# colmap/glomap

Measured on NVIDIA B200. Metric: observations/sec per BA LM-iteration, higher is better.
Workload: dtype f64

## Files before the change

### glomap_b200/csrc/ba_kernels.cuh

```cuda
#pragma once
#include "common.cuh"
#include "pcg.cuh"

namespace b200 {

constexpr int kCamRec = 8;
constexpr int kIntrRec = 8;
constexpr double kZEps = 1e-12;
constexpr int kSeg = 256;
constexpr int kIntrSmem = 16;
constexpr int kJpDoubles = 6;
constexpr int kJcDoubles = 9;
constexpr int kSensorRec = 16;

struct BAView {
  int C, P, K;
  long long N;
  int n_tiles;
  int n_segs;
  int min_views;
  const int* obs_cam;
  const int* obs_pt;
  const double2* obs_xy;
  const unsigned* pt_begin;
// ... 489 lines not shown
  }
  const double d = U[(size_t)c * 21 + sym_idx(6, k, k)];
  const double js2 = js * js;
  Dc[i] = fmin(fmax(d * js2, 1e-6), 1e32) / (radius * js2);
}

__device__ __forceinline__ void point_damping(const double* V6, const double* js, double radius, double Dp[3]) {
  const double d[3] = {V6[0], V6[3], V6[5]};
#pragma unroll
  for (int k = 0; k < 3; ++k) {
    const double js2 = js[k] * js[k];
    Dp[k] = fmin(fmax(d[k] * js2, 1e-6), 1e32) / (radius * js2);
  }
}
__global__ void ba_damp_points(int P, const double* __restrict__ V, double* __restrict__ jscale_p, int set_jscale,
                               double radius, double* __restrict__ Vinv) {
  const int p = blockIdx.x * blockDim.x + threadIdx.x;
  if (p >= P) return;
  double v6[6];
#pragma unroll
  for (int k = 0; k < 6; ++k) v6[k] = V[6 * (size_t)p + k];
  double js[3];
  if (set_jscale) {
    js[0] = 1.0 / (1.0 + sqrt(v6[0]));
    js[1] = 1.0 / (1.0 + sqrt(v6[3]));
    js[2] = 1.0 / (1.0 + sqrt(v6[5]));
#pragma unroll
    for (int k = 0; k < 3; ++k) jscale_p[3 * (size_t)p + k] = js[k];
  } else {
#pragma unroll
    for (int k = 0; k < 3; ++k) js[k] = jscale_p[3 * (size_t)p + k];
  }
  double Dp[3];
  point_damping(v6, js, radius, Dp);
  v6[0] += Dp[0];
  v6[3] += Dp[1];
  v6[5] += Dp[2];
  double inv[6];
  sym3_inverse(v6, inv);
#pragma unroll
  for (int k = 0; k < 6; ++k) Vinv[6 * (size_t)p + k] = inv[k];
}

__global__ void __launch_bounds__(128) ba_schur_diag(BAView v) {
  const int warp = (blockIdx.x * blockDim.x + threadIdx.x) >> 5;
  const int lane = threadIdx.x & 31;
  if (warp >= v.n_segs) return;
  const int cam = v.seg_cam[warp];
  const int b = v.seg_begin[warp], e = v.seg_end[warp];
  double S[21];
#pragma unroll
  for (int k = 0; k < 21; ++k) S[k] = 0.0;
  for (int i = b + lane; i < e; i += 32) {
    const int o = v.camord_obs[i];
    const int pt = v.pt_c[i];
    double w[18], vi[6];
// ... 392 lines not shown
```

### glomap_b200/csrc/ba_kernels_v2.cuh

```cuda
#pragma once
#include "ba_kernels.cuh"
#include "pcg.cuh"

namespace b200 {

struct BAViewV2 {
  const double* Ap;
  double* Ac;
  double* z4;
  double* Bc = nullptr;
  double* Ufk = nullptr;
  const IntrVarRec* ivar = nullptr;
  int C = 0;
};

template <int NK>
__device__ __forceinline__ void obs_intr_rows(const ObsCore& o, const double* __restrict__ ir, const IntrVarRec& iv,
                                              const double Jp[6], double Jk[2][NK > 0 ? NK : 1],
                                              double B[NK > 0 ? 3 * NK : 1]) {
#pragma unroll
  for (int j = 0; j < NK; ++j) {
    double jx = 0.0, jy = 0.0;
    if (j < iv.mb) intr_param_jac(ir, iv.pidx[j], o.uv[0], o.uv[1], 1.0, jx, jy);
    if (!o.valid) jx = jy = 0.0;
// ... 187 lines not shown
      }
    }
  }
#pragma unroll
  for (int k = 0; k < 21; ++k) {
    const double s = warp_sum(U[k]);
    if (lane == k && s != 0.0) atomicAdd(&v.U[(size_t)cam * 21 + k], s);
  }
#pragma unroll
  for (int k = 0; k < 6; ++k) {
    const double s = warp_sum(g[k]);
    if (lane == 21 + k && s != 0.0) atomicAdd(&v.gc[(size_t)cam * 6 + k], s);
  }
}

__global__ void __launch_bounds__(128) ba2_schur_diag(BAView v, BAViewV2 v2, const double* __restrict__ cam_rec) {
  const int warp = (blockIdx.x * blockDim.x + threadIdx.x) >> 5;
  const int lane = threadIdx.x & 31;
  if (warp >= v.n_segs) return;
  const int cam = v.seg_cam[warp];
  const int b = v.seg_begin[warp], e = v.seg_end[warp];
  double RR[6] = {0, 0, 0, 0, 0, 0}, RT[9] = {0, 0, 0, 0, 0, 0, 0, 0, 0}, TT[6] = {0, 0, 0, 0, 0, 0};
  const double* row = v2.Ac + (size_t)(v.seg_row0[warp] >> 5) * (kJcDoubles * 32) + lane;
  for (int i = b + lane; i < e; i += 32, row += kJcDoubles * 32) {
    const double A[6] = {ld_stream(row), ld_stream(row + 32), ld_stream(row + 64), ld_stream(row + 96), ld_stream(row + 128),
                         ld_stream(row + 160)};
    const double X[3] = {ld_stream(row + 192), ld_stream(row + 224), ld_stream(row + 256)};
    const int pt = ld_stream(v.pt_c + i);
    const double2* vp = reinterpret_cast<const double2*>(v.Vinv + (size_t)pt * 6);
    const double2 v0 = vp[0], v1 = vp[1], v2_ = vp[2];
    const double vi[6] = {v0.x, v0.y, v1.x, v1.y, v2_.x, v2_.y};
    const double Ac0[3] = {A[0], A[1], A[2]}, Ac1[3] = {A[1], A[3], A[4]}, Ac2[3] = {A[2], A[4], A[5]};
    double T0[3], T1[3], T2[3];
    sym3_mul(vi, Ac0, T0);
    sym3_mul(vi, Ac1, T1);
    sym3_mul(vi, Ac2, T2);
    double N[3][3];
    {
      double c0[3], c1[3], c2[3];
      sym3_mul(A, T0, c0);
      sym3_mul(A, T1, c1);
      sym3_mul(A, T2, c2);
#pragma unroll
      for (int r = 0; r < 3; ++r) { N[r][0] = c0[r]; N[r][1] = c1[r]; N[r][2] = c2[r]; }
    }
// ... 14 lines not shown
    }
    RR[0] += -2.0 * PK[0][0]; RR[1] += -2.0 * PK[0][1]; RR[2] += -2.0 * PK[0][2];
    RR[3] += -2.0 * PK[1][1]; RR[4] += -2.0 * PK[1][2]; RR[5] += -2.0 * PK[2][2];
#pragma unroll
    for (int r = 0; r < 3; ++r)
#pragma unroll
      for (int c = 0; c < 3; ++c) RT[3 * r + c] += P[r][c];
    TT[0] += N[0][0]; TT[1] += N[0][1]; TT[2] += N[0][2]; TT[3] += N[1][1]; TT[4] += N[1][2]; TT[5] += N[2][2];
  }
#pragma unroll
  for (int k = 0; k < 6; ++k) RR[k] = warp_sum(RR[k]);
#pragma unroll
  for (int k = 0; k < 9; ++k) RT[k] = warp_sum(RT[k]);
#pragma unroll
  for (int k = 0; k < 6; ++k) TT[k] = warp_sum(TT[k]);
  if (lane == 0) {
    const double4 q4c = ld_rec32(cam_rec + (size_t)cam * kCamRec);
    const double4 t4c = ld_rec32(cam_rec + (size_t)cam * kCamRec + 4);
    const int mask = (int)(__double_as_longlong(t4c.w) & 0xff);
    const double q[4] = {q4c.x, q4c.y, q4c.z, q4c.w};
    double R[9];
    quat_to_R(q, R);
    double M[6][6];
    const double rr[3][3] = {{RR[0], RR[1], RR[2]}, {RR[1], RR[3], RR[4]}, {RR[2], RR[4], RR[5]}};
    const double tt[3][3] = {{TT[0], TT[1], TT[2]}, {TT[1], TT[3], TT[4]}, {TT[2], TT[4], TT[5]}};
    for (int r = 0; r < 3; ++r)
      for (int c = 0; c < 3; ++c) {
        M[r][c] = rr[r][c];
        M[3 + r][3 + c] = tt[r][c];
        M[r][3 + c] = RT[3 * r + c];
        M[3 + c][r] = RT[3 * r + c];
      }
    double T[6][6];
    for (int blk = 0; blk < 2; ++blk)
      for (int r = 0; r < 3; ++r)
        for (int c = 0; c < 6; ++c)
          T[3 * blk + r][c] = R[3 * r] * M[3 * blk][c] + R[3 * r + 1] * M[3 * blk + 1][c] + R[3 * r + 2] * M[3 * blk + 2][c];
// ... 170 lines not shown
  for (long long r = (long long)blockIdx.x * blockDim.x + threadIdx.x; r < rows; r += (long long)gridDim.x * blockDim.x) {
    const double2* row = reinterpret_cast<const double2*>(part + 4 * r);
    const double2 u = row[0], w = row[1];
    a0 += u.x; a1 += u.y; a2 += w.x; a3 += w.y;
  }
  a0 = block_sum(a0, scratch);
  a1 = block_sum(a1, scratch);
  a2 = block_sum(a2, scratch);
  a3 = block_sum(a3, scratch);
  if (threadIdx.x == 0) {
    double* o = out + 4 * (size_t)blockIdx.x;
    o[0] = a0; o[1] = a1; o[2] = a2; o[3] = a3;
  }
}

__global__ void ba2_point_rhs_z(BAView v, BAViewV2 v2) {
  const int p = blockIdx.x * blockDim.x + threadIdx.x;
  if (p >= v.P) return;
  double vi[6], g[3], z[3];
#pragma unroll
  for (int k = 0; k < 6; ++k) vi[k] = v.Vinv[6 * (size_t)p + k];
#pragma unroll
  for (int k = 0; k < 3; ++k) g[k] = v.gp[3 * (size_t)p + k];
  sym3_mul(vi, g, z);
  const bool pvalid = (int)(v.pt_begin[p + 1] - v.pt_begin[p]) >= v.min_views;
  *reinterpret_cast<double4*>(v2.z4 + 4 * (size_t)p) = pvalid ? make_double4(z[0], z[1], z[2], 0.0) : make_double4(0, 0, 0, 0);
}

template <int NK>
__global__ void __launch_bounds__(128, B200_PB_MIN_CTAS) ba2_pass_b(BAView v, BAViewV2 v2, const double* __restrict__ cam_rec,
                                                 double* __restrict__ y, const PcgCtl* __restrict__ ctl, int seg_lo,
                                                 int seg_hi) {
  if (ctl && ctl->done) return;
  const int warp = seg_lo + ((blockIdx.x * blockDim.x + threadIdx.x) >> 5);
  const int lane = threadIdx.x & 31;
  if (warp >= seg_hi) return;
  const int cam = v.seg_cam[warp];
  const int b = v.seg_begin[warp], e = v.seg_end[warp];
  double acc[6] = {0, 0, 0, 0, 0, 0};
  constexpr int NKK = NK > 0 ? NK : 1;
  double accK[NKK];
#pragma unroll
  for (int k = 0; k < NKK; ++k) accK[k] = 0.0;
// ... 157 lines not shown
```

### glomap_b200/csrc/ba_kernels_v3.cuh

```cuda
#pragma once
#include "ba_kernels_v2.cuh"

namespace b200 {

constexpr int kEllWindow = 1024;
constexpr int kEllThreads = 128;

struct EllView {
  int n_groups;
  const int* row0;
  const int* pt;
  const int* len;
  const int* cam;
  const double2* xy;
  const unsigned short* sensor;
  double* A;
  double* B = nullptr;
};

template <class Sort>
__global__ void __launch_bounds__(kEllWindow) ell_sort_window(int P, int min_views, const unsigned* __restrict__ pt_begin,
                                                              int* __restrict__ ell_pt, int* __restrict__ ell_len,
                                                              int* __restrict__ ell_slot, int* __restrict__ group_rows) {
  __shared__ typename Sort::TempStorage tmp;
// ... 181 lines not shown
#pragma unroll
      for (int k = 0; k < 3; ++k) {
        v.gp[3 * (size_t)pt + k] = gp[k];
        gmax = fmax(gmax, fabs(gp[k]));
      }
    }
  }
  cost = warp_sum(cost);
  gmax = warp_max(gmax);
  if (lane == 0) {
    part_cost[slot >> 5] = cost;
    part_gmax[slot >> 5] = gmax;
  }
}

__global__ void __launch_bounds__(kEllThreads) ba3_cost(BAView v, EllView ell, const double* __restrict__ cam_rec,
                                                         const double* __restrict__ intr_rec,
                                                         const double* __restrict__ points, double huber_a,
                                                         double* __restrict__ part_cost) {
  __shared__ double scratch[32];
  const int slot = blockIdx.x * kEllThreads + threadIdx.x;
  const int lane = threadIdx.x & 31;
  const int g = slot >> 5;
  double cost = 0.0;
  if (g < ell.n_groups) {
    const int pt = ell.pt[slot];
    const int mylen = ell.len[slot];
    const int r0 = ell.row0[g], nrow = ell.row0[g + 1] - r0;
    double X0 = 0, X1 = 0, X2 = 0;
    if (pt >= 0) {
      X0 = points[3 * (size_t)pt]; X1 = points[3 * (size_t)pt + 1]; X2 = points[3 * (size_t)pt + 2];
    }
#pragma unroll 2
    for (int j = 0; j < nrow; ++j) {
      if (j >= mylen) continue;
      const size_t idx = ((size_t)r0 + j) * 32 + lane;
      const int cam = ld_stream(ell.cam + idx);
      const double2 xy = ld_stream(ell.xy + idx);
      const double4 q4 = ld_rec32(cam_rec + (size_t)cam * kCamRec);
      const double4 t4 = ld_rec32(cam_rec + (size_t)cam * kCamRec + 4);
      const double* sr = ell.sensor ? v.sensor_rec + (size_t)ell.sensor[idx] * kSensorRec : nullptr;
      const double* ir = intr_rec + (size_t)obs_intr_idx(t4, sr) * kIntrRec;
      const double q[4] = {q4.x, q4.y, q4.z, q4.w};
      double R[9];
      quat_to_R(q, R);
      double xc = R[0] * X0 + R[1] * X1 + R[2] * X2 + t4.x;
      double yc = R[3] * X0 + R[4] * X1 + R[5] * X2 + t4.y;
      double zc = R[6] * X0 + R[7] * X1 + R[8] * X2 + t4.z;
      if (sr) sensor_apply(sr, xc, yc, zc);
      if (zc > kZEps) {
        double px, py;
        project_only(ir, xc, yc, zc, px, py);
        const double e0 = px - xy.x, e1 = py - xy.y;
        double rho0, rho1;
        huber(e0 * e0 + e1 * e1, huber_a, rho0, rho1);
        cost += 0.5 * rho0;
      }
    }
  }
  cost = block_sum(cost, scratch);
  if (threadIdx.x == 0) part_cost[blockIdx.x] = cost;
}

__global__ void __launch_bounds__(1024) ba3_reduce_partials(int n, const double* __restrict__ part_a,
                                                           const double* __restrict__ part_b, double* __restrict__ out_sum,
                                                           double* __restrict__ out_max) {
  __shared__ double scratch[32];
  double s = 0.0, m = 0.0;
  for (int i = threadIdx.x; i < n; i += blockDim.x) {
    s += part_a[i];
    if (part_b) m = fmax(m, part_b[i]);
  }
  s = block_sum(s, scratch);
  if (threadIdx.x == 0) *out_sum = s;
  if (part_b) {
    m = block_max(m, scratch);
    if (threadIdx.x == 0) *out_max = m;
  }
}

template <int MODE, int NK>
__global__ void __launch_bounds__(kEllThreads, MODE == 0 ? B200_EA_MIN_CTAS : B200_EA2_MIN_CTAS) ba3_pass_a(
    BAView v, EllView ell, BAViewV2 v2, const double* __restrict__ xp, const double* __restrict__ points,
    double* __restrict__ points_new, double radius, double* __restrict__ bscal, const PcgCtl* __restrict__ ctl) {
  __shared__ double scratch[32];
  if (ctl && ctl->done) return;
  const int slot = blockIdx.x * kEllThreads + threadIdx.x;
  const int lane = threadIdx.x & 31;
  const int g = slot >> 5;
  double b0 = 0, b1 = 0, b2 = 0, b3 = 0;
  if (g < ell.n_groups) {
    const int pt = ell.pt[slot];
// ... 93 lines not shown
```

### glomap_b200/csrc/ba_solver.cuh

```cuda
#pragma once
#include <cub/cub.cuh>

#include <algorithm>
#include <cmath>
#include <cstdlib>
#include <vector>

#include "ba_kernels.cuh"
#include "ba_kernels_v2.cuh"
#include "ba_kernels_v3.cuh"
#include "ba_kernels_ext.cuh"
#include "filter_kernels.cuh"
#include "processor_kernels.cuh"
#include "context.cuh"
#include "pcg.cuh"

namespace b200 {

__global__ void k_expand_obs_pt(int P, const unsigned* __restrict__ pt_begin, int* __restrict__ obs_pt) {
  const int p = blockIdx.x * blockDim.x + threadIdx.x;
  if (p >= P) return;
  for (unsigned o = pt_begin[p]; o < pt_begin[p + 1]; ++o) obs_pt[o] = p;
}
__global__ void k_cam_keys(long long N, int VC, int smul, int min_views, const int* __restrict__ obs_cam,
// ... 107 lines not shown
  std::vector<unsigned char> h_sensor_var;
  DevBuf<unsigned char> sensor_var;
  DevBuf<double> sens_q[2], sens_t[2], sens_q_saved, sens_t_saved;
  b200::ExtView ext_view() {
    b200::ExtView e;
    e.C = C; e.K = K; e.S = S; e.ivar = ivar.p; e.sensor_var = (ext_s && S > 0) ? sensor_var.p : nullptr;
    return e;
  }
  bool use_v2 = false;
  bool use_ell = false;
  int ell_groups = 0, ell_ctas = 0, ell_bpart_rows = 0;
  long long ell_rows = 0;
  DevBuf<int> ell_row0, ell_pt, ell_len, ell_slot, ell_cam;
  DevBuf<double2> ell_xy;
  DevBuf<unsigned short> ell_sensor;
  DevBuf<double> ell_A, ell_part;
  b200::EllView ell_view() {
    b200::EllView e;
    e.n_groups = ell_groups; e.row0 = ell_row0.p; e.pt = ell_pt.p; e.len = ell_len.p; e.cam = ell_cam.p; e.xy = ell_xy.p;
    e.sensor = S > 0 ? ell_sensor.p : nullptr; e.A = ell_A.p; e.B = kfast ? ell_B.p : nullptr;
    return e;
  }
  DevBuf<double> Jc, z4, xq, bpart, bpart2;
  size_t smem_k3v2 = 0;
  bool kfast = false;
  int nk = 0;
  DevBuf<double> ell_B, Bc, Ufk;
  b200::BAViewV2 view2() {
    b200::BAViewV2 w;
    w.Ap = W.p; w.Ac = Jc.p; w.z4 = z4.p;
    w.Bc = kfast ? Bc.p : nullptr; w.Ufk = kfast ? Ufk.p : nullptr; w.ivar = ivar.p; w.C = C;
// ... 193 lines not shown
      size_t need = 0;
      cub::DeviceScan::ExclusiveSum(nullptr, need, grows.p, ell_row0.p, ell_groups + 1, s);
      DevBuf<unsigned char> tmp3;
      tmp3.alloc(need + 16);
      size_t tb3 = tmp3.bytes();
      cub::DeviceScan::ExclusiveSum(tmp3.p, tb3, grows.p, ell_row0.p, ell_groups + 1, s);
      ctx->launches += 1;
      int h_rows = 0;
      B200_CUDA_OK(cudaMemcpyAsync(&h_rows, ell_row0.p + ell_groups, sizeof(int), cudaMemcpyDeviceToHost, s));
      B200_CUDA_OK(cudaStreamSynchronize(s));
      ell_rows = h_rows;
      const size_t cells = (size_t)std::max<long long>(ell_rows, 1) * 32;
      ell_cam.alloc(cells); ell_xy.alloc(cells); ell_A.alloc(cells * 6);
      if (S > 0) ell_sensor.alloc(cells);
      ell_part.alloc((size_t)ell_ctas * (kEllThreads / 32) * 2 + 8);
      ell_bpart_rows = ell_ctas;
      B200_LAUNCH(ctx, ell_scatter_obs, cdiv(N, 256), 256, 0, N, min_views, obs_pt.p, pt_begin.p, obs_cam.p, obs_xy.p,
                  S > 0 ? obs_sensor.p : nullptr, ell_slot.p, ell_row0.p, ell_cam.p, ell_xy.p, S > 0 ? ell_sensor.p : nullptr);
      B200_CUDA_OK(cudaStreamSynchronize(s));
    }
    for (int i = 0; i < 2; ++i) {
      quat[i].alloc((size_t)C * 4); trans[i].alloc((size_t)C * 3); points[i].alloc((size_t)P * 3);
    }
    intr.alloc((size_t)K * B200SFM_INTR_STRIDE);
    intr_cand.alloc((size_t)K * B200SFM_INTR_STRIDE);
    cam_rec.alloc((size_t)C * kCamRec); intr_rec.alloc((size_t)K * kIntrRec);
    W.alloc((size_t)N * kWDoubles); V.alloc((size_t)P * 6); Vinv.alloc((size_t)P * 6); gp.alloc((size_t)P * 3);
    lin.alloc((size_t)CB * 27 + 1 + (size_t)ctx->world);
    Sd.alloc((size_t)CB * 27);
    Minv.alloc((size_t)CB * 21);
// ... 83 lines not shown
    if (S > 0)
      B200_LAUNCH(ctx, bax_build_sensor_rec, cdiv(S, 256), 256, 0, S, sens_q[which].p, sens_t[which].p,
                  sensor_intr.p, sensor_rec.p);
  }
  void set_sensor_variable(const uint8_t* h_var) {
    h_sensor_var.assign(h_var, h_var + S);
    sensor_var.upload(h_sensor_var.data(), S, ctx->stream);
    B200_CUDA_OK(cudaStreamSynchronize(ctx->stream));
  }
  void get_sensor_poses(double* h_q, double* h_t) {
    if (h_q) sens_q[cur].download(h_q, (size_t)S * 4, ctx->stream);
    if (h_t) sens_t[cur].download(h_t, (size_t)S * 3, ctx->stream);
    B200_CUDA_OK(cudaStreamSynchronize(ctx->stream));
  }

  void launch_cost(int which, double huber_a) {
    using namespace b200;
    if (use_ell) {
      B200_LAUNCH(ctx, ba3_cost, ell_ctas, kEllThreads, 0, view(), ell_view(), cam_rec.p, intr_rec.p, points[which].p, huber_a, ell_part.p);
      B200_LAUNCH(ctx, ba3_reduce_partials, 1, 256, 0, ell_ctas, ell_part.p, nullptr, scal.p + 6, nullptr);
    } else {
      const int grid = std::min(cdiv(N, 256), 148 * 8);
      B200_LAUNCH(ctx, ba_cost, grid, 256, 0, view(), cam_rec.p, intr_rec.p, points[which].p, huber_a, scal.p + 6);
    }
  }

  double eval_cost(int which, double huber_a) {
    using namespace b200;
    build_records(which);
    B200_CUDA_OK(cudaMemsetAsync(scal.p + 6, 0, sizeof(double), ctx->stream));
    launch_cost(which, huber_a);
    ctx->allreduce_sum(scal.p + 6, 1);
    B200_CUDA_OK(cudaMemcpyAsync(ctx->h_scal, scal.p + 6, sizeof(double), cudaMemcpyDeviceToHost, ctx->stream));
    B200_CUDA_OK(cudaStreamSynchronize(ctx->stream));
    return ctx->h_scal[0];
// ... 9 lines not shown
    cudaEvent_t e0 = nullptr, e1 = nullptr;
    if (profile) {
      e0 = timer_lin.next();
      e1 = timer_lin.next();
      B200_CUDA_OK(cudaEventRecord(e0, s));
    }
    if (use_ell) {
      const int nwp = ell_ctas * (kEllThreads / 32);
#define B200_LIN_P(NKV)                                                                                                   \
  B200_LAUNCH(ctx, ba3_linearize_points<NKV>, ell_ctas, kEllThreads, 0, v, ell_view(), cam_rec.p, intr_rec.p, points[cur].p, \
              huber_a, points_var ? 1 : 0, ell_part.p, ell_part.p + nwp, ivar.p)
      if (kfast && nk == 2) B200_LIN_P(2);
      else if (kfast && nk == 1) B200_LIN_P(1);
      else B200_LIN_P(0);
#undef B200_LIN_P
      B200_LAUNCH(ctx, ba3_reduce_partials, 1, 1024, 0, nwp, ell_part.p, ell_part.p + nwp, scal.p, scal.p + 1);
    } else if (use_v2)
      B200_LAUNCH(ctx, ba_linearize_points<true>, n_tiles, kTile, smem_k1, v, cam_rec.p, intr_rec.p, points[cur].p, huber_a,
                  points_var ? 1 : 0, scal.p);
    else
      B200_LAUNCH(ctx, ba_linearize_points<false>, n_tiles, kTile, smem_k1, v, cam_rec.p, intr_rec.p, points[cur].p, huber_a,
                  points_var ? 1 : 0, scal.p);
    if (profile) B200_CUDA_OK(cudaEventRecord(e1, s));
    if (n_segs > 0) {
      const int sgrid = cdiv((long long)n_segs * 32, 128);
      if (kfast) {
        Ufk.zero(s);
        B200_LAUNCH(ctx, ba2_pad_points, cdiv(P, 256), 256, 0, P, points[cur].p, z4.p);
        if (nk == 2) B200_LAUNCH(ctx, ba2_linearize_cams<2>, sgrid, 128, 0, v, view2(), cam_rec.p, intr_rec.p, points[cur].p, huber_a);
        else B200_LAUNCH(ctx, ba2_linearize_cams<1>, sgrid, 128, 0, v, view2(), cam_rec.p, intr_rec.p, points[cur].p, huber_a);
      } else if (ext) {
// ... 157 lines not shown
      else if (ext_s) B200_EXT_B(false, true);
      else B200_EXT_B(false, false);
#undef B200_EXT_B
    }
  }

  void launch_pass_b(const b200::BAView& v, double* y, const b200::PcgCtl* ctl, int seg_lo = 0, int seg_hi = -1) {
    using namespace b200;
    if (seg_hi < 0) seg_hi = n_segs;
    if (seg_hi <= seg_lo) return;
    const int grid = cdiv((long long)(seg_hi - seg_lo) * 32, 128);
    if (kfast && nk == 2) B200_LAUNCH(ctx, ba2_pass_b<2>, grid, 128, 0, v, view2(), cam_rec.p, y, ctl, seg_lo, seg_hi);
    else if (kfast) B200_LAUNCH(ctx, ba2_pass_b<1>, grid, 128, 0, v, view2(), cam_rec.p, y, ctl, seg_lo, seg_hi);
    else B200_LAUNCH(ctx, ba2_pass_b<0>, grid, 128, 0, v, view2(), cam_rec.p, y, ctl, seg_lo, seg_hi);
  }
  void launch_pass_a0(const b200::BAView& v, double radius, const b200::PcgCtl* ctl) {
    using namespace b200;
    if (kfast && nk == 2)
      B200_LAUNCH(ctx, (ba3_pass_a<0, 2>), ell_ctas, kEllThreads, 0, v, ell_view(), view2(), xq.p, points[cur].p, nullptr, radius, nullptr, ctl);
    else if (kfast)
      B200_LAUNCH(ctx, (ba3_pass_a<0, 1>), ell_ctas, kEllThreads, 0, v, ell_view(), view2(), xq.p, points[cur].p, nullptr, radius, nullptr, ctl);
    else
      B200_LAUNCH(ctx, (ba3_pass_a<0, 0>), ell_ctas, kEllThreads, 0, v, ell_view(), view2(), xq.p, points[cur].p, nullptr, radius, nullptr, ctl);
  }
  void launch_cross(const double* x, double* y, const b200::PcgCtl* ctl) {
    using namespace b200;
    if (nk == 2) B200_LAUNCH(ctx, ba2k_cross<2>, cdiv(C, 256), 256, 0, C, K, cam_rec.p, Ufk.p, x, y, ctl);
    else B200_LAUNCH(ctx, ba2k_cross<1>, cdiv(C, 256), 256, 0, C, K, cam_rec.p, Ufk.p, x, y, ctl);
  }

  StepResult compute_step(const b200sfm_ba_opts& o, double radius, bool points_var, bool set_jscale_p, bool profile) {
    using namespace b200;
    cudaStream_t s = ctx->stream;
    BAView v = view();
    const int nB6 = nbk * 6;
    if (points_var) B200_LAUNCH(ctx, ba_damp_points, cdiv(P, 256), 256, 0, P, V.p, jscale_p.p, set_jscale_p ? 1 : 0, radius, Vinv.p);
    B200_LAUNCH(ctx, ba_damp_cams, cdiv(nB6, 256), 256, 0, nbk, U(), jscale_c.p, radius, Dc.p);
    const bool recomp = ext && !kfast;
    const bool schur_jacobi = points_var && o.preconditioner == 1 && !recomp;
    double* yrhs = Sd.p + (size_t)CB * 21;
    Sd.zero(s);
    if (schur_jacobi && n_segs > 0) {
      if (use_v2) B200_LAUNCH(ctx, ba2_schur_diag, cdiv((long long)n_segs * 32, 128), 128, 0, v, view2(), cam_rec.p);
      else B200_LAUNCH(ctx, ba_schur_diag, cdiv((long long)n_segs * 32, 128), 128, 0, v);
    }
    if (points_var) {
      if (use_v2) {
        B200_LAUNCH(ctx, ba2_point_rhs_z, cdiv(P, 256), 256, 0, v, view2());
        if (recomp) ext_matvec(nullptr, yrhs, o.thres_loss_function, radius, true, nullptr);
        else if (n_segs > 0) launch_pass_b(v, yrhs, nullptr);
      } else {
        B200_LAUNCH(ctx, ba_schur_pass<1>, n_tiles, kTile, smem_k3, v, nullptr, yrhs, nullptr, nullptr, radius, nullptr);
      }
    } else if (recomp) {
      z4.zero(s);
    }
    if (schur_jacobi || points_var) ctx->allreduce_sum(Sd.p, (size_t)CB * 27);
    B200_LAUNCH(ctx, ba_build_precond, cdiv(nbk, 128), 128, 0, nbk, U(), Dc.p, schur_jacobi ? Sd.p : nullptr, Minv.p);
    B200_LAUNCH(ctx, k_rhs, cdiv(nB6, 256), 256, 0, nB6, gc(), points_var ? yrhs : nullptr, bvec.p);
    const int max_it = std::max(1, o.pcg_max_iterations);
    const int nblk = cdiv(nbk, kPcgThreads);
    ctx->pcgh.ensure(max_it, (size_t)nblk * 3, ctx->world);
    double* part_pq = ctx->pcgh.d_part;
    double* part_rz = ctx->pcgh.d_part + nblk;
// ... 272 lines not shown
```

### glomap_b200/csrc/common.cuh

```cuda
#pragma once
#include <cuda_runtime.h>
#include <stdint.h>
#include <stdio.h>

#include <string>

namespace b200 {

#ifndef B200_TILE
#define B200_TILE 128
#endif
#ifndef B200_K1_MIN_CTAS
#define B200_K1_MIN_CTAS 5
#endif
#ifndef B200_K3_MIN_CTAS
#define B200_K3_MIN_CTAS 8
#endif
#ifndef B200_PA_MIN_CTAS
#define B200_PA_MIN_CTAS 12
#endif
#ifndef B200_LC_MIN_CTAS
#define B200_LC_MIN_CTAS 3
#endif
#ifndef B200_PB_PREFETCH
#define B200_PB_PREFETCH 1
#endif
#ifndef B200_PB_MIN_CTAS
#define B200_PB_MIN_CTAS 7
#endif
#ifndef B200_E1_MIN_CTAS
#define B200_E1_MIN_CTAS 4
#endif
#ifndef B200_E1_PIPE
#define B200_E1_PIPE 1
#endif
#ifndef B200_EA_MIN_CTAS
#define B200_EA_MIN_CTAS 8
#endif
#ifndef B200_EA2_MIN_CTAS
#define B200_EA2_MIN_CTAS 6
#endif
#ifndef B200_STREAM_HINTS
#define B200_STREAM_HINTS 1
// ... 278 lines not shown
```

### profiles/sass_excerpt.py

```python
#!/usr/bin/env python
import collections
import os
import re
import subprocess

ROOT = os.path.dirname(os.path.dirname(os.path.abspath(__file__)))
KERNELS = ["ba3_linearize_points", "ba2_linearize_cams", "ba3_pass_a", "ba2_pass_b", "ba2_schur_diag", "ba3_cost",
           "ba2_pcg_direction_pack", "pcg_update", "pcg_apply_diag", "bax_pass_b", "ba2k_cross", "gp_schur_pass", "ra_laplacian_csr",
           "ra2_laplacian_dot", "ra2_coarse", "p2p_allreduce_sum", "proc_undistort", "trk_hook"]
KEEP = re.compile(r"^(LDG|STG|LDS|STS|RED|ATOM|BAR|SHFL|DFMA|DMUL|DADD|MUFU|CCTL|UBLKCP|SYNCS|MEMBAR|ERRBAR|LDGSTS)")


def main():
    lib = os.path.join(ROOT, "glomap_b200", "libb200sfm.so")
    txt = subprocess.run(["cuobjdump", "-sass", lib], capture_output=True, text=True).stdout
    names = subprocess.run(["cu++filt"], input="\n".join(re.findall(r"Function : (\S+)", txt)), capture_output=True, text=True).stdout.split("\n")
    mangled = re.findall(r"Function : (\S+)", txt)
    demangle = dict(zip(mangled, names))
    cur, counts, totals = None, collections.defaultdict(collections.Counter), collections.Counter()
    for line in txt.splitlines():
        m = re.search(r"Function : (\S+)", line)
        if m:
            cur = demangle.get(m.group(1), m.group(1))
            continue
# ... 20 lines not shown
```

Measured before the change: 2.252 billion.

## Fuse Schur RHS into diagonal pass, fold point z into damping, parallelize partial reductions

Point z = Vinv*g is now computed inside the point damping kernel, and the Schur-diagonal kernel also accumulates the reduced camera and intrinsic RHS from z, so the separate point-RHS kernel and a second sweep over camera rows go away. The cost kernel gains software prefetching of the next camera records and observations, reduces per warp instead of per block, and has a min-CTA launch bound. The single-CTA partial reduction becomes a multi-CTA reduction with a last-block finish driven by an atomic counter. These changes add register pressure and atomics, and the counter must be reset correctly between calls.

```diff
diff --git a/glomap_b200/csrc/ba_kernels.cuh b/glomap_b200/csrc/ba_kernels.cuh
--- a/glomap_b200/csrc/ba_kernels.cuh
+++ b/glomap_b200/csrc/ba_kernels.cuh
@@ -527,7 +527,9 @@
   }
 }
 __global__ void ba_damp_points(int P, const double* __restrict__ V, double* __restrict__ jscale_p, int set_jscale,
-                               double radius, double* __restrict__ Vinv) {
+                               double radius, double* __restrict__ Vinv, const double* __restrict__ gp = nullptr,
+                               const unsigned* __restrict__ pt_begin = nullptr, int min_views = 0,
+                               double* __restrict__ z4 = nullptr) {
   const int p = blockIdx.x * blockDim.x + threadIdx.x;
   if (p >= P) return;
   double v6[6];
@@ -553,6 +555,14 @@
   sym3_inverse(v6, inv);
 #pragma unroll
   for (int k = 0; k < 6; ++k) Vinv[6 * (size_t)p + k] = inv[k];
+  if (z4) {
+    double g[3], z[3];
+#pragma unroll
+    for (int k = 0; k < 3; ++k) g[k] = gp[3 * (size_t)p + k];
+    sym3_mul(inv, g, z);
+    const bool pvalid = (int)(pt_begin[p + 1] - pt_begin[p]) >= min_views;
+    *reinterpret_cast<double4*>(z4 + 4 * (size_t)p) = pvalid ? make_double4(z[0], z[1], z[2], 0.0) : make_double4(0, 0, 0, 0);
+  }
 }
 
 __global__ void __launch_bounds__(128) ba_schur_diag(BAView v) {
diff --git a/glomap_b200/csrc/ba_kernels_v2.cuh b/glomap_b200/csrc/ba_kernels_v2.cuh
--- a/glomap_b200/csrc/ba_kernels_v2.cuh
+++ b/glomap_b200/csrc/ba_kernels_v2.cuh
@@ -225,21 +225,59 @@
   }
 }
 
-__global__ void __launch_bounds__(128) ba2_schur_diag(BAView v, BAViewV2 v2, const double* __restrict__ cam_rec) {
+template <int NK>
+__global__ void __launch_bounds__(128, B200_SR_MIN_CTAS) ba2_schur_rhs(BAView v, BAViewV2 v2, const double* __restrict__ cam_rec,
+                                                                     double* __restrict__ y) {
   const int warp = (blockIdx.x * blockDim.x + threadIdx.x) >> 5;
   const int lane = threadIdx.x & 31;
   if (warp >= v.n_segs) return;
   const int cam = v.seg_cam[warp];
   const int b = v.seg_begin[warp], e = v.seg_end[warp];
   double RR[6] = {0, 0, 0, 0, 0, 0}, RT[9] = {0, 0, 0, 0, 0, 0, 0, 0, 0}, TT[6] = {0, 0, 0, 0, 0, 0};
-  const double* row = v2.Ac + (size_t)(v.seg_row0[warp] >> 5) * (kJcDoubles * 32) + lane;
-  for (int i = b + lane; i < e; i += 32, row += kJcDoubles * 32) {
+  double acc[6] = {0, 0, 0, 0, 0, 0};
+  constexpr int NKK = NK > 0 ? NK : 1;
+  double accK[NKK];
+#pragma unroll
+  for (int k = 0; k < NKK; ++k) accK[k] = 0.0;
+  const double* row0 = v2.Ac + (size_t)(v.seg_row0[warp] >> 5) * (kJcDoubles * 32) + lane;
+  const double* rowB0 = NK > 0 ? v2.Bc + (size_t)(v.seg_row0[warp] >> 5) * (3 * NK * 32) + lane : nullptr;
+  const uint64_t keep = l2_policy_evict_last();
+  int ptr[kSeg / 32];
+#pragma unroll
+  for (int j = 0; j < kSeg / 32; ++j) {
+    const int i = b + lane + 32 * j;
+    ptr[j] = i < e ? ld_stream(v.pt_c + i) : -1;
+  }
+#pragma unroll
+  for (int j = 0; j < kSeg / 32; ++j) {
+    if (b + 32 * j >= e) break;
+    const int pt = ptr[j];
+    if (pt < 0) continue;
+    const double* row = row0 + (size_t)j * (kJcDoubles * 32);
     const double A[6] = {ld_stream(row), ld_stream(row + 32), ld_stream(row + 64), ld_stream(row + 96), ld_stream(row + 128),
                          ld_stream(row + 160)};
     const double X[3] = {ld_stream(row + 192), ld_stream(row + 224), ld_stream(row + 256)};
-    const int pt = ld_stream(v.pt_c + i);
     const double2* vp = reinterpret_cast<const double2*>(v.Vinv + (size_t)pt * 6);
     const double2 v0 = vp[0], v1 = vp[1], v2_ = vp[2];
+    const double4 z = ld_keep4(v2.z4 + 4 * (size_t)pt, keep);
+    if (NK > 0) {
+      const double* bp = rowB0 + (size_t)j * (3 * NK * 32);
+#pragma unroll
+      for (int k = 0; k < NK; ++k)
+        accK[k] += ld_stream(bp + 32 * (3 * k)) * z.x + ld_stream(bp + 32 * (3 * k + 1)) * z.y +
+                   ld_stream(bp + 32 * (3 * k + 2)) * z.z;
+    }
+    {
+      const double w0 = A[0] * z.x + A[1] * z.y + A[2] * z.z;
+      const double w1 = A[1] * z.x + A[3] * z.y + A[4] * z.z;
+      const double w2 = A[2] * z.x + A[4] * z.y + A[5] * z.z;
+      acc[0] += 2.0 * (X[1] * w2 - X[2] * w1);
+      acc[1] += 2.0 * (X[2] * w0 - X[0] * w2);
+      acc[2] += 2.0 * (X[0] * w1 - X[1] * w0);
+      acc[3] += w0;
+      acc[4] += w1;
+      acc[5] += w2;
+    }
     const double vi[6] = {v0.x, v0.y, v1.x, v1.y, v2_.x, v2_.y};
     const double Ac0[3] = {A[0], A[1], A[2]}, Ac1[3] = {A[1], A[3], A[4]}, Ac2[3] = {A[2], A[4], A[5]};
     double T0[3], T1[3], T2[3];
@@ -284,13 +322,30 @@
   for (int k = 0; k < 9; ++k) RT[k] = warp_sum(RT[k]);
 #pragma unroll
   for (int k = 0; k < 6; ++k) TT[k] = warp_sum(TT[k]);
+#pragma unroll
+  for (int k = 0; k < 6; ++k) acc[k] = warp_sum(acc[k]);
+  if (NK > 0) {
+    const size_t kb = (size_t)(v2.C + v.seg_intr[warp]);
+#pragma unroll
+    for (int k = 0; k < NK; ++k) {
+      const double sk = warp_sum(accK[k]);
+      if (lane == 0 && sk != 0.0) atomicAdd(&y[kb * 6 + k], -sk);
+    }
+  }
+  if (lane >= 6) return;
+  const double4 q4c = ld_rec32(cam_rec + (size_t)cam * kCamRec);
+  const double4 t4c = ld_rec32(cam_rec + (size_t)cam * kCamRec + 4);
+  const int mask = (int)(__double_as_longlong(t4c.w) & 0xff);
+  const double q[4] = {q4c.x, q4c.y, q4c.z, q4c.w};
+  double R[9];
+  quat_to_R(q, R);
+  {
+    const int blk = lane / 3, r = lane % 3;
+    const bool fixed = blk == 0 ? (mask & 1) : (mask & 2);
+    const double s = R[3 * r] * acc[3 * blk] + R[3 * r + 1] * acc[3 * blk + 1] + R[3 * r + 2] * acc[3 * blk + 2];
+    if (!fixed && s != 0.0) atomicAdd(&y[(size_t)cam * 6 + lane], -s);
+  }
   if (lane == 0) {
-    const double4 q4c = ld_rec32(cam_rec + (size_t)cam * kCamRec);
-    const double4 t4c = ld_rec32(cam_rec + (size_t)cam * kCamRec + 4);
-    const int mask = (int)(__double_as_longlong(t4c.w) & 0xff);
-    const double q[4] = {q4c.x, q4c.y, q4c.z, q4c.w};
-    double R[9];
-    quat_to_R(q, R);
     double M[6][6];
     const double rr[3][3] = {{RR[0], RR[1], RR[2]}, {RR[1], RR[3], RR[4]}, {RR[2], RR[4], RR[5]}};
     const double tt[3][3] = {{TT[0], TT[1], TT[2]}, {TT[1], TT[3], TT[4]}, {TT[2], TT[4], TT[5]}};
@@ -491,19 +546,6 @@
   }
 }
 
-__global__ void ba2_point_rhs_z(BAView v, BAViewV2 v2) {
-  const int p = blockIdx.x * blockDim.x + threadIdx.x;
-  if (p >= v.P) return;
-  double vi[6], g[3], z[3];
-#pragma unroll
-  for (int k = 0; k < 6; ++k) vi[k] = v.Vinv[6 * (size_t)p + k];
-#pragma unroll
-  for (int k = 0; k < 3; ++k) g[k] = v.gp[3 * (size_t)p + k];
-  sym3_mul(vi, g, z);
-  const bool pvalid = (int)(v.pt_begin[p + 1] - v.pt_begin[p]) >= v.min_views;
-  *reinterpret_cast<double4*>(v2.z4 + 4 * (size_t)p) = pvalid ? make_double4(z[0], z[1], z[2], 0.0) : make_double4(0, 0, 0, 0);
-}
-
 template <int NK>
 __global__ void __launch_bounds__(128, B200_PB_MIN_CTAS) ba2_pass_b(BAView v, BAViewV2 v2, const double* __restrict__ cam_rec,
                                                  double* __restrict__ y, const PcgCtl* __restrict__ ctl, int seg_lo,
diff --git a/glomap_b200/csrc/ba_kernels_v3.cuh b/glomap_b200/csrc/ba_kernels_v3.cuh
--- a/glomap_b200/csrc/ba_kernels_v3.cuh
+++ b/glomap_b200/csrc/ba_kernels_v3.cuh
@@ -219,11 +219,10 @@
   }
 }
 
-__global__ void __launch_bounds__(kEllThreads) ba3_cost(BAView v, EllView ell, const double* __restrict__ cam_rec,
-                                                         const double* __restrict__ intr_rec,
-                                                         const double* __restrict__ points, double huber_a,
-                                                         double* __restrict__ part_cost) {
-  __shared__ double scratch[32];
+__global__ void __launch_bounds__(kEllThreads, B200_EC_MIN_CTAS) ba3_cost(BAView v, EllView ell, const double* __restrict__ cam_rec,
+                                                                          const double* __restrict__ intr_rec,
+                                                                          const double* __restrict__ points, double huber_a,
+                                                                          double* __restrict__ part_cost) {
   const int slot = blockIdx.x * kEllThreads + threadIdx.x;
   const int lane = threadIdx.x & 31;
   const int g = slot >> 5;
@@ -236,51 +235,92 @@
     if (pt >= 0) {
       X0 = points[3 * (size_t)pt]; X1 = points[3 * (size_t)pt + 1]; X2 = points[3 * (size_t)pt + 2];
     }
-#pragma unroll 2
+    int camB = 0;
+    double2 xyA = make_double2(0, 0), xyB = xyA;
+    double4 qA = make_double4(0, 0, 0, 1), tA = make_double4(0, 0, 0, 0);
+    if (mylen > 0) {
+      const size_t i0 = (size_t)r0 * 32 + lane;
+      const int camA = ld_stream(ell.cam + i0);
+      xyA = ld_stream(ell.xy + i0);
+      if (mylen > 1) {
+        camB = ld_stream(ell.cam + i0 + 32);
+        xyB = ld_stream(ell.xy + i0 + 32);
+      }
+      qA = ld_rec32(cam_rec + (size_t)camA * kCamRec);
+      tA = ld_rec32(cam_rec + (size_t)camA * kCamRec + 4);
+    }
     for (int j = 0; j < nrow; ++j) {
-      if (j >= mylen) continue;
+      if (j >= mylen) break;
       const size_t idx = ((size_t)r0 + j) * 32 + lane;
-      const int cam = ld_stream(ell.cam + idx);
-      const double2 xy = ld_stream(ell.xy + idx);
-      const double4 q4 = ld_rec32(cam_rec + (size_t)cam * kCamRec);
-      const double4 t4 = ld_rec32(cam_rec + (size_t)cam * kCamRec + 4);
+      double4 qB = qA, tB = tA;
+      int camC = 0;
+      double2 xyC = xyB;
+      if (j + 1 < mylen) {
+        qB = ld_rec32(cam_rec + (size_t)camB * kCamRec);
+        tB = ld_rec32(cam_rec + (size_t)camB * kCamRec + 4);
+      }
+      if (j + 2 < mylen) {
+        camC = ld_stream(ell.cam + idx + 64);
+        xyC = ld_stream(ell.xy + idx + 64);
+      }
       const double* sr = ell.sensor ? v.sensor_rec + (size_t)ell.sensor[idx] * kSensorRec : nullptr;
-      const double* ir = intr_rec + (size_t)obs_intr_idx(t4, sr) * kIntrRec;
-      const double q[4] = {q4.x, q4.y, q4.z, q4.w};
+      const double* ir = intr_rec + (size_t)obs_intr_idx(tA, sr) * kIntrRec;
+      const double q[4] = {qA.x, qA.y, qA.z, qA.w};
       double R[9];
       quat_to_R(q, R);
-      double xc = R[0] * X0 + R[1] * X1 + R[2] * X2 + t4.x;
-      double yc = R[3] * X0 + R[4] * X1 + R[5] * X2 + t4.y;
-      double zc = R[6] * X0 + R[7] * X1 + R[8] * X2 + t4.z;
+      double xc = R[0] * X0 + R[1] * X1 + R[2] * X2 + tA.x;
+      double yc = R[3] * X0 + R[4] * X1 + R[5] * X2 + tA.y;
+      double zc = R[6] * X0 + R[7] * X1 + R[8] * X2 + tA.z;
       if (sr) sensor_apply(sr, xc, yc, zc);
       if (zc > kZEps) {
         double px, py;
         project_only(ir, xc, yc, zc, px, py);
-        const double e0 = px - xy.x, e1 = py - xy.y;
+        const double e0 = px - xyA.x, e1 = py - xyA.y;
         double rho0, rho1;
         huber(e0 * e0 + e1 * e1, huber_a, rho0, rho1);
         cost += 0.5 * rho0;
       }
-    }
-  }
-  cost = block_sum(cost, scratch);
-  if (threadIdx.x == 0) part_cost[blockIdx.x] = cost;
-}
-
-__global__ void __launch_bounds__(1024) ba3_reduce_partials(int n, const double* __restrict__ part_a,
-                                                           const double* __restrict__ part_b, double* __restrict__ out_sum,
-                                                           double* __restrict__ out_max) {
+      qA = qB; tA = tB; xyA = xyB; xyB = xyC; camB = camC;
+    }
+  }
+  cost = warp_sum(cost);
+  if (lane == 0) part_cost[slot >> 5] = cost;
+}
+
+constexpr int kSumCtas = 296;
+__global__ void __launch_bounds__(256) ba3_sum_partials(int n, const double* __restrict__ part_a, const double* __restrict__ part_b,
+                                                        double* __restrict__ stage, unsigned* __restrict__ counter,
+                                                        double* __restrict__ out_sum, double* __restrict__ out_max) {
   __shared__ double scratch[32];
+  __shared__ bool last;
   double s = 0.0, m = 0.0;
-  for (int i = threadIdx.x; i < n; i += blockDim.x) {
+  for (int i = blockIdx.x * blockDim.x + threadIdx.x; i < n; i += gridDim.x * blockDim.x) {
     s += part_a[i];
     if (part_b) m = fmax(m, part_b[i]);
   }
   s = block_sum(s, scratch);
-  if (threadIdx.x == 0) *out_sum = s;
-  if (part_b) {
-    m = block_max(m, scratch);
-    if (threadIdx.x == 0) *out_max = m;
+  if (part_b) m = block_max(m, scratch);
+  if (threadIdx.x == 0) {
+    stage[blockIdx.x] = s;
+    if (part_b) stage[gridDim.x + blockIdx.x] = m;
+    __threadfence();
+    last = atomicAdd(counter, 1u) == gridDim.x - 1;
+  }
+  __syncthreads();
+  if (!last) return;
+  __threadfence();
+  s = 0.0;
+  m = 0.0;
+  for (int i = threadIdx.x; i < (int)gridDim.x; i += blockDim.x) {
+    s += __ldcg(stage + i);
+    if (part_b) m = fmax(m, __ldcg(stage + gridDim.x + i));
+  }
+  s = block_sum(s, scratch);
+  if (part_b) m = block_max(m, scratch);
+  if (threadIdx.x == 0) {
+    *out_sum = s;
+    if (part_b) *out_max = m;
+    *counter = 0u;
   }
 }
 
diff --git a/glomap_b200/csrc/ba_solver.cuh b/glomap_b200/csrc/ba_solver.cuh
--- a/glomap_b200/csrc/ba_solver.cuh
+++ b/glomap_b200/csrc/ba_solver.cuh
@@ -145,7 +145,8 @@
   DevBuf<int> ell_row0, ell_pt, ell_len, ell_slot, ell_cam;
   DevBuf<double2> ell_xy;
   DevBuf<unsigned short> ell_sensor;
-  DevBuf<double> ell_A, ell_part;
+  DevBuf<double> ell_A, ell_part, ell_stage;
+  DevBuf<unsigned> ell_count;
   b200::EllView ell_view() {
     b200::EllView e;
     e.n_groups = ell_groups; e.row0 = ell_row0.p; e.pt = ell_pt.p; e.len = ell_len.p; e.cam = ell_cam.p; e.xy = ell_xy.p;
@@ -369,6 +370,9 @@
       ell_cam.alloc(cells); ell_xy.alloc(cells); ell_A.alloc(cells * 6);
       if (S > 0) ell_sensor.alloc(cells);
       ell_part.alloc((size_t)ell_ctas * (kEllThreads / 32) * 2 + 8);
+      ell_stage.alloc(2 * (size_t)kSumCtas);
+      ell_count.alloc(1);
+      ell_count.zero(s);
       ell_bpart_rows = ell_ctas;
       B200_LAUNCH(ctx, ell_scatter_obs, cdiv(N, 256), 256, 0, N, min_views, obs_pt.p, pt_begin.p, obs_cam.p, obs_xy.p,
                   S > 0 ? obs_sensor.p : nullptr, ell_slot.p, ell_row0.p, ell_cam.p, ell_xy.p, S > 0 ? ell_sensor.p : nullptr);
@@ -482,11 +486,17 @@
     B200_CUDA_OK(cudaStreamSynchronize(ctx->stream));
   }
 
+  void reduce_partials(int n, const double* part_a, const double* part_b, double* out_sum, double* out_max) {
+    using namespace b200;
+    const int nb = std::max(1, std::min(cdiv(n, 256), kSumCtas));
+    B200_LAUNCH(ctx, ba3_sum_partials, nb, 256, 0, n, part_a, part_b, ell_stage.p, ell_count.p, out_sum, out_max);
+  }
+
   void launch_cost(int which, double huber_a) {
     using namespace b200;
     if (use_ell) {
       B200_LAUNCH(ctx, ba3_cost, ell_ctas, kEllThreads, 0, view(), ell_view(), cam_rec.p, intr_rec.p, points[which].p, huber_a, ell_part.p);
-      B200_LAUNCH(ctx, ba3_reduce_partials, 1, 256, 0, ell_ctas, ell_part.p, nullptr, scal.p + 6, nullptr);
+      reduce_partials(ell_ctas * (kEllThreads / 32), ell_part.p, nullptr, scal.p + 6, nullptr);
     } else {
       const int grid = std::min(cdiv(N, 256), 148 * 8);
       B200_LAUNCH(ctx, ba_cost, grid, 256, 0, view(), cam_rec.p, intr_rec.p, points[which].p, huber_a, scal.p + 6);
@@ -526,7 +536,7 @@
       else if (kfast && nk == 1) B200_LIN_P(1);
       else B200_LIN_P(0);
 #undef B200_LIN_P
-      B200_LAUNCH(ctx, ba3_reduce_partials, 1, 1024, 0, nwp, ell_part.p, ell_part.p + nwp, scal.p, scal.p + 1);
+      reduce_partials(nwp, ell_part.p, ell_part.p + nwp, scal.p, scal.p + 1);
     } else if (use_v2)
       B200_LAUNCH(ctx, ba_linearize_points<true>, n_tiles, kTile, smem_k1, v, cam_rec.p, intr_rec.p, points[cur].p, huber_a,
                   points_var ? 1 : 0, scal.p);
@@ -714,6 +724,13 @@
     else if (kfast) B200_LAUNCH(ctx, ba2_pass_b<1>, grid, 128, 0, v, view2(), cam_rec.p, y, ctl, seg_lo, seg_hi);
     else B200_LAUNCH(ctx, ba2_pass_b<0>, grid, 128, 0, v, view2(), cam_rec.p, y, ctl, seg_lo, seg_hi);
   }
+  void launch_schur_rhs(const b200::BAView& v, double* y) {
+    using namespace b200;
+    const int grid = cdiv((long long)n_segs * 32, 128);
+    if (kfast && nk == 2) B200_LAUNCH(ctx, ba2_schur_rhs<2>, grid, 128, 0, v, view2(), cam_rec.p, y);
+    else if (kfast) B200_LAUNCH(ctx, ba2_schur_rhs<1>, grid, 128, 0, v, view2(), cam_rec.p, y);
+    else B200_LAUNCH(ctx, ba2_schur_rhs<0>, grid, 128, 0, v, view2(), cam_rec.p, y);
+  }
   void launch_pass_a0(const b200::BAView& v, double radius, const b200::PcgCtl* ctl) {
     using namespace b200;
     if (kfast && nk == 2)
@@ -734,20 +751,20 @@
     cudaStream_t s = ctx->stream;
     BAView v = view();
     const int nB6 = nbk * 6;
-    if (points_var) B200_LAUNCH(ctx, ba_damp_points, cdiv(P, 256), 256, 0, P, V.p, jscale_p.p, set_jscale_p ? 1 : 0, radius, Vinv.p);
+    if (points_var)
+      B200_LAUNCH(ctx, ba_damp_points, cdiv(P, 256), 256, 0, P, V.p, jscale_p.p, set_jscale_p ? 1 : 0, radius, Vinv.p, gp.p,
+                  pt_begin.p, min_views, use_v2 ? z4.p : nullptr);
     B200_LAUNCH(ctx, ba_damp_cams, cdiv(nB6, 256), 256, 0, nbk, U(), jscale_c.p, radius, Dc.p);
     const bool recomp = ext && !kfast;
     const bool schur_jacobi = points_var && o.preconditioner == 1 && !recomp;
     double* yrhs = Sd.p + (size_t)CB * 21;
     Sd.zero(s);
-    if (schur_jacobi && n_segs > 0) {
-      if (use_v2) B200_LAUNCH(ctx, ba2_schur_diag, cdiv((long long)n_segs * 32, 128), 128, 0, v, view2(), cam_rec.p);
-      else B200_LAUNCH(ctx, ba_schur_diag, cdiv((long long)n_segs * 32, 128), 128, 0, v);
-    }
+    if (schur_jacobi && !use_v2 && n_segs > 0)
+      B200_LAUNCH(ctx, ba_schur_diag, cdiv((long long)n_segs * 32, 128), 128, 0, v);
     if (points_var) {
       if (use_v2) {
-        B200_LAUNCH(ctx, ba2_point_rhs_z, cdiv(P, 256), 256, 0, v, view2());
         if (recomp) ext_matvec(nullptr, yrhs, o.thres_loss_function, radius, true, nullptr);
+        else if (schur_jacobi && n_segs > 0) launch_schur_rhs(v, yrhs);
         else if (n_segs > 0) launch_pass_b(v, yrhs, nullptr);
       } else {
         B200_LAUNCH(ctx, ba_schur_pass<1>, n_tiles, kTile, smem_k3, v, nullptr, yrhs, nullptr, nullptr, radius, nullptr);
diff --git a/glomap_b200/csrc/common.cuh b/glomap_b200/csrc/common.cuh
--- a/glomap_b200/csrc/common.cuh
+++ b/glomap_b200/csrc/common.cuh
@@ -27,6 +27,12 @@
 #endif
 #ifndef B200_PB_MIN_CTAS
 #define B200_PB_MIN_CTAS 7
+#endif
+#ifndef B200_SR_MIN_CTAS
+#define B200_SR_MIN_CTAS 4
+#endif
+#ifndef B200_EC_MIN_CTAS
+#define B200_EC_MIN_CTAS 6
 #endif
 #ifndef B200_E1_MIN_CTAS
 #define B200_E1_MIN_CTAS 4
diff --git a/profiles/lm_phase_times.py b/profiles/lm_phase_times.py
--- /dev/null
+++ b/profiles/lm_phase_times.py
@@ -0,0 +1,148 @@
+#!/usr/bin/env python
+import argparse
+import json
+import os
+import subprocess
+import sys
+import tempfile
+import time
+
+import numpy as np
+
+ROOT = os.path.dirname(os.path.dirname(os.path.abspath(__file__)))
+sys.path.insert(0, ROOT)
+FIELDS = ["quat", "trans", "points", "pt_obs_begin", "obs_cam", "obs_xy", "cam_intr", "intr_model", "intr_params"]
+
+
+def gpu_info() -> str:
+    try:
+        out = subprocess.run(["nvidia-smi", "--query-gpu=name,power.limit", "--format=csv,noheader"], capture_output=True,
+                             text=True, timeout=30).stdout.strip().splitlines()
+        return out[0].strip() if out else "unknown"
+    except (OSError, subprocess.TimeoutExpired):
+        return "unknown"
+
+
+def gen(cache: str) -> None:
+    from glomap_b200 import synthetic as S
+    t0 = time.time()
+    sc = S.make_scene(10_000, 2_000_000, 10.0, seed=1, pixel_sigma=0.5, chunk=50_000)
+    init = S.perturb_scene(sc, chunk=50_000)
+    for f in FIELDS:
+        np.save(os.path.join(cache, f"{f}.npy"), getattr(sc, f))
+    for f in ("quat", "trans", "points"):
+        np.save(os.path.join(cache, f"init_{f}.npy"), getattr(init, f))
+    print(f"scene generated in {time.time() - t0:.1f} s, N = {sc.N}", flush=True)
+
+
+def worker(args) -> dict:
+    import torch
+    from torch.autograd import DeviceType
+    from torch.profiler import ProfilerActivity, profile
+    from glomap_b200 import estimators as E, synthetic as S
+
+    cache = args.cache
+    sc = S.Scene(*[np.load(os.path.join(cache, f"{f}.npy")) for f in FIELDS])
+    init = {f: np.load(os.path.join(cache, f"init_{f}.npy")) for f in ("quat", "trans", "points")}
+    torch.cuda.set_device(0)
+    ctx = E.default_context()
+    opts = E.BundleAdjusterOptions(optimize_intrinsics=bool(args.optimize_intrinsics), profile_kernels=True, design=0)
+    opts.solver_options.max_num_iterations = 20
+    opts.solver_options.pcg_rel_tolerance = 0.05
+    opts.solver_options.pcg_max_iterations = 200
+    prob = E.BAProblem(ctx, sc, 3, E.first_frame_mask(sc.C))
+    prob.set_state(sc.intr_params, init["quat"], init["trans"], init["points"])
+    prob.save_state()
+    for _ in range(args.warmup):
+        prob.restore_state()
+        prob.solve(opts)
+    torch.cuda.synchronize()
+    stats = []
+    with profile(activities=[ProfilerActivity.CUDA]) as prof:
+        for _ in range(args.solves):
+            prob.restore_state()
+            stats.append(prob.solve(opts))
+        torch.cuda.synchronize()
+    per = {}
+    for ev in prof.events():
+        if ev.device_type != DeviceType.CUDA:
+            continue
+        d = per.setdefault(ev.name, [0, 0.0])
+        d[0] += 1
+        d[1] += ev.time_range.elapsed_us()
+    n = args.solves
+    lm = sum(s.iterations for s in stats)
+    pcg = sum(s.pcg_iterations for s in stats)
+    rows = sorted(({"name": k, "launches_per_solve": c / n, "us_per_solve": t / n, "us_per_launch": t / max(c, 1)}
+                   for k, (c, t) in per.items()), key=lambda r: -r["us_per_solve"])
+    return {"lib": os.environ.get("B200SFM_LIB", "glomap_b200/libb200sfm.so"), "gpu": gpu_info(),
+            "optimize_intrinsics": int(args.optimize_intrinsics), "solves": n,
+            "ms_per_solve_events": float(np.mean([s.ms_total for s in stats])),
+            "lm_iterations_per_solve": lm / n, "pcg_iterations_per_lm_iteration": pcg / max(lm, 1),
+            "kernel_launches_per_solve": sum(s.kernel_launches for s in stats) / n,
+            "final_cost": stats[-1].final_cost, "kernels": rows}
+
+
+def table(res: dict) -> str:
+    lm = res["lm_iterations_per_solve"]
+    lines = [f"### `{res['lib']}`", "",
+             f"GPU: {res['gpu']} (name, power limit).  {res['solves']} profiled solves; "
+             f"{res['ms_per_solve_events']:.2f} ms per solve (CUDA events of the solver, profiler attached), "
+             f"{lm:g} LM iterations, {res['pcg_iterations_per_lm_iteration']:.2f} PCG iterations per LM iteration, "
+             f"{res['kernel_launches_per_solve']:g} launches per solve (solver count), final cost {res['final_cost']:.9e}.", "",
+             "| kernel | launches / solve | µs / solve | µs / LM iteration | µs / launch |", "|---|---|---|---|---|"]
+    tot = 0.0
+    for r in res["kernels"]:
+        tot += r["us_per_solve"]
+        lines.append(f"| `{r['name'][:90]}` | {r['launches_per_solve']:g} | {r['us_per_solve']:.1f} | "
+                     f"{r['us_per_solve'] / max(lm, 1):.1f} | {r['us_per_launch']:.1f} |")
+    lines.append(f"| **sum of device times** | {sum(r['launches_per_solve'] for r in res['kernels']):g} | {tot:.1f} | "
+                 f"{tot / max(lm, 1):.1f} | |")
+    return "\n".join(lines) + "\n"
+
+
+def main() -> None:
+    ap = argparse.ArgumentParser(description=__doc__, formatter_class=argparse.RawDescriptionHelpFormatter)
+    ap.add_argument("--libs", default="", help="comma-separated libb200sfm.so paths (default: the tree's build)")
+    ap.add_argument("--solves", type=int, default=3, help="profiled solves per library")
+    ap.add_argument("--warmup", type=int, default=2, help="unprofiled warm-up solves per library")
+    ap.add_argument("--optimize-intrinsics", type=int, default=0, help="1: bench.py's second line (focal lengths refined)")
+    ap.add_argument("--out", default=None, help="directory for lm_phase_times.{json,md}")
+    ap.add_argument("--worker", action="store_true", help=argparse.SUPPRESS)
+    ap.add_argument("--cache", default=None, help=argparse.SUPPRESS)
+    args = ap.parse_args()
+    if args.solves < 1 or args.warmup < 0:
+        raise SystemExit("--solves must be >= 1 and --warmup >= 0")
+    if args.worker:
+        print("RESULT " + json.dumps(worker(args)), flush=True)
+        return
+    libs = [os.path.abspath(x) for x in args.libs.split(",") if x] or [None]
+    for lib in libs:
+        if lib is not None and not os.path.exists(lib):
+            raise SystemExit(f"{lib} not found")
+    results = []
+    with tempfile.TemporaryDirectory(prefix="b200sfm_phase_") as cache:
+        gen(cache)
+        for lib in libs:
+            env = dict(os.environ)
+            if lib is not None:
+                env["B200SFM_LIB"] = lib
+            cmd = [sys.executable, os.path.abspath(__file__), "--worker", "--cache", cache, "--solves", str(args.solves),
+                   "--warmup", str(args.warmup), "--optimize-intrinsics", str(args.optimize_intrinsics)]
+            p = subprocess.run(cmd, env=env, capture_output=True, text=True)
+            line = [ln for ln in p.stdout.splitlines() if ln.startswith("RESULT ")]
+            if p.returncode != 0 or not line:
+                sys.stderr.write(p.stdout[-4000:] + p.stderr[-4000:])
+                raise SystemExit(f"worker for {lib} failed (exit {p.returncode})")
+            results.append(json.loads(line[-1][len("RESULT "):]))
+            print(table(results[-1]), flush=True)
+    if args.out:
+        os.makedirs(args.out, exist_ok=True)
+        with open(os.path.join(args.out, "lm_phase_times.json"), "w") as f:
+            json.dump(results, f, indent=1)
+        with open(os.path.join(args.out, "lm_phase_times.md"), "w") as f:
+            f.write("\n".join(table(r) for r in results))
+
+
+if __name__ == "__main__":
+    main()
diff --git a/profiles/sass_excerpt.py b/profiles/sass_excerpt.py
--- a/profiles/sass_excerpt.py
+++ b/profiles/sass_excerpt.py
@@ -5,7 +5,7 @@
 import subprocess
 
 ROOT = os.path.dirname(os.path.dirname(os.path.abspath(__file__)))
-KERNELS = ["ba3_linearize_points", "ba2_linearize_cams", "ba3_pass_a", "ba2_pass_b", "ba2_schur_diag", "ba3_cost",
+KERNELS = ["ba3_linearize_points", "ba2_linearize_cams", "ba3_pass_a", "ba2_pass_b", "ba2_schur_rhs", "ba3_cost",
            "ba2_pcg_direction_pack", "pcg_update", "pcg_apply_diag", "bax_pass_b", "ba2k_cross", "gp_schur_pass", "ra_laplacian_csr",
            "ra2_laplacian_dot", "ra2_coarse", "p2p_allreduce_sum", "proc_undistort", "trk_hook"]
 KEEP = re.compile(r"^(LDG|STG|LDS|STS|RED|ATOM|BAR|SHFL|DFMA|DMUL|DADD|MUFU|CCTL|UBLKCP|SYNCS|MEMBAR|ERRBAR|LDGSTS)")
```

New measurement: 2.314 billion (median of 6 runs). 1.03x the previous value.
